# kvcache-ai/ktransformers

Hardware: NVIDIA H100
Metric: decode tok/s DeepSeek-V3 671B INT4 (Q4_K_M) MoE-block hot path; HBM GB/s vs roofline (higher is better)
Workload: dtype int8xint4/int6->int32 dp4a, fp32 scales+accumulate, bf16 in/out

## Files before the change

### include/ktb200.h

```cpp
#ifndef KTB200_H
#define KTB200_H
#include <stddef.h>
#include <stdint.h>
#ifdef __cplusplus
extern "C" {
#endif

#define KTB200_OK 0
#define KTB200_EINVAL (-1)
#define KTB200_ECUDA (-2)
#define KTB200_ESTATE (-3)
#define KTB200_ENOMEM (-4)

enum ktb200_ggml_type {
    KTB200_TYPE_F32 = 0, KTB200_TYPE_F16 = 1, KTB200_TYPE_Q8_0 = 8, KTB200_TYPE_Q2_K = 10,
    KTB200_TYPE_Q3_K = 11, KTB200_TYPE_Q4_K = 12, KTB200_TYPE_Q5_K = 13, KTB200_TYPE_Q6_K = 14,
    KTB200_TYPE_Q8_K = 15, KTB200_TYPE_IQ4_XS = 23, KTB200_TYPE_BF16 = 30,
    KTB200_TYPE_IQ2_XXS = 16, KTB200_TYPE_IQ1_S = 19,
    KTB200_TYPE_RAWINT4_G32 = 256
};

const char* ktb200_last_error(void);
const char* ktb200_version(void);
long ktb200_type_size(int ggml_type);
// ... 149 lines not shown
    void* out;
} ktb200_mla_prefill_params;
int ktb200_mla_prefill(const ktb200_mla_prefill_params* p, void* stream);
void ktb200_debug_grouped(long long* trace_dev);

int ktb200_add_rmsnorm(void* residual_dev, const void* delta_dev, const void* weight_dev, float eps, void* out_dev, int n_tokens,
                       int hidden, void* stream);
int ktb200_mla_prep(const void* q_dev, int num_heads, int qk_nope_head_dim, const void* kv_a_out_dev, const void* kv_a_norm_weight_dev,
                    float eps, const float* cos_dev, const float* sin_dev, void* kv_cache_dev, int page_size, const int* page_idx_dev,
                    const int* page_offset_dev, void* q_pe_out_dev, int n_tokens, void* stream);

int ktb200_mla_absorb_q(const void* q_dev, long q_head_stride, long q_token_stride, const void* w_uk_dev, int num_heads, int qk_nope_head_dim,
                        int kv_lora_rank, void* q_abs_out_dev, int n_tokens, void* stream);
int ktb200_mla_absorb_o(const void* attn_latent_dev, const void* w_uv_dev, int num_heads, int v_head_dim, int kv_lora_rank, void* out_dev,
                        int n_tokens, void* stream);

int ktb200_mla_kv_write(void* kv_cache, int page_size, const void* ckv, const void* k_pe, const int* page_idx,
                        const int* page_offset, int n_tokens, void* stream);

int ktb200_debug_stream_read(const void* src_dev, long bytes, int mode, int unroll, int ctas_per_sm, int chunk_bytes,
                             void* stream, float* ms_out);
void ktb200_debug_block_trace(unsigned long long* trace_dev);
long ktb200_debug_block_sync_words(ktb200_moe* moe, unsigned* host_out, long n);

#ifdef __cplusplus
}
#endif
#endif
```

### ktransformers_b200/csrc/common.cuh

```cuda
#pragma once
#include <cuda_bf16.h>
#include <cuda_fp16.h>
#include <cuda_runtime.h>
#include <stdint.h>

#include "../../include/ktb200.h"

#define QK_K 256
#define SZ_Q8_0 34
#define SZ_Q2_K 84
#define SZ_Q3_K 110
#define SZ_Q4_K 144
#define SZ_Q5_K 176
#define SZ_Q6_K 210
#define SZ_Q8_K 292
#define SZ_IQ4_XS 136
#define SZ_IQ2_XXS 66
#define SZ_IQ1_S 50
#define SZ_RAWINT4 144

namespace ktb {

void set_error(const char* fmt, ...);
void count_launch(int n = 1);
// ... 70 lines not shown
__host__ __device__ inline bool is_hidden_type(int t) {
    return t == KTB200_TYPE_F32 || t == KTB200_TYPE_F16 || t == KTB200_TYPE_BF16;
}
__host__ __device__ inline long row_bytes(long n, int t) { return n / blck_size(t) * type_size(t); }

#ifdef __CUDACC__
__device__ __forceinline__ uint4 ldg_stream16(const void* p) {
    uint4 r;
    asm volatile("ld.global.nc.L1::no_allocate.v4.u32 {%0, %1, %2, %3}, [%4];"
                 : "=r"(r.x), "=r"(r.y), "=r"(r.z), "=r"(r.w)
                 : "l"(p));
    return r;
}
__device__ __forceinline__ uint32_t ldg_stream4(const void* p) {
    uint32_t r;
    asm volatile("ld.global.nc.L1::no_allocate.u32 %0, [%1];" : "=r"(r) : "l"(p));
    return r;
}
__device__ __forceinline__ void prefetch_l2_bulk(const void* p, uint32_t bytes) {
    asm volatile("cp.async.bulk.prefetch.L2.global [%0], %1;" ::"l"(p), "r"(bytes) : "memory");
}
__device__ __forceinline__ void griddep_launch_dependents() { asm volatile("griddepcontrol.launch_dependents;" ::: "memory"); }
__device__ __forceinline__ void griddep_wait() { asm volatile("griddepcontrol.wait;" ::: "memory"); }
__device__ __forceinline__ uint16_t ldg_u16(const void* p) { return __ldg(reinterpret_cast<const unsigned short*>(p)); }
__device__ __forceinline__ uint8_t ldg_u8(const void* p) { return __ldg(reinterpret_cast<const unsigned char*>(p)); }

__device__ __forceinline__ int dp4a_s8s8(uint32_t a, uint32_t b, int c) { return __dp4a((int)a, (int)b, c); }
__device__ __forceinline__ int dp4a_u8s8(uint32_t a, uint32_t b, int c) {
    int d;
    asm("dp4a.u32.s32 %0, %1, %2, %3;" : "=r"(d) : "r"(a), "r"(b), "r"(c));
    return d;
}

__device__ __forceinline__ float warp_sum(float v) {
#pragma unroll
    for (int o = 16; o > 0; o >>= 1) v += __shfl_xor_sync(0xffffffffu, v, o);
    return v;
}

__device__ __forceinline__ float fp16_bits_to_f32(uint16_t h) { return __half2float(__ushort_as_half(h)); }

__device__ __forceinline__ uint16_t f32_to_bf16_ggml(float f) {
    uint32_t i = __float_as_uint(f);
    if ((i & 0x7fffffffu) > 0x7f800000u) return (uint16_t)((i >> 16) | 64);
    if (!(i & 0x7f800000u)) return (uint16_t)((i & 0x80000000u) >> 16);
    return (uint16_t)((i + (0x7fffu + ((i >> 16) & 1))) >> 16);
// ... 45 lines not shown
```

### ktransformers_b200/csrc/gate.cuh

```cuda
#pragma once
#include "common.cuh"

namespace ktb {

constexpr int kGateWarps = 4;
constexpr int kGateThreads = kGateWarps * 32;
constexpr int kGateTokTile = 8;

struct GateParams {
    const float* W;
    const void* x;
    int hidden_type, E, H, T, S;
    int top_k, n_group, topk_group, scoring, topk_method, norm_topk_prob;
    float routed_scaling_factor;
    const float* bias;
    float* partial;
    float* logits_out;
    int64_t* idx;
    float* w;
    const int* bsz;
    unsigned* ticket;
};

static inline int gate_splits(int E, int H, int nsms) {
// ... 6 lines not shown

__device__ __forceinline__ unsigned fkey(float f) {
    const unsigned u = __float_as_uint(f);
    return (u & 0x80000000u) ? ~u : (u | 0x80000000u);
}

constexpr int kGateEPT = 4;

__device__ __forceinline__ float fkey_inv(unsigned k) {
    return __uint_as_float((k & 0x80000000u) ? (k & 0x7fffffffu) : ~k);
}

template <int BAR>
__device__ __forceinline__ void gate_sync() {
    if (BAR == 0) __syncthreads();
    else asm volatile("bar.sync %0, %1;" ::"n"(BAR), "n"(kGateThreads) : "memory");
}
struct GateSel {
    int E, S, top_k, n_group, topk_group, scoring, topk_method, norm_topk_prob;
    float routed_scaling_factor;
    const float* bias;
    const float* partial;
};
template <int BAR>
__device__ void gate_select_token(const GateParams& pin, int t, float* sm, int64_t* idx_out, float* w_out, float* logits_out) {
    const GateSel p{pin.E, pin.S, pin.top_k, pin.n_group, pin.topk_group, pin.scoring, pin.topk_method, pin.norm_topk_prob,
                    pin.routed_scaling_factor, pin.bias, pin.partial};
    const int E = p.E, tid = threadIdx.x, lane = tid & 31, warp = tid >> 5;
    float* scores = sm;
    float* choice = sm + E;
    float* gsc = choice + E;
    unsigned* wbest = reinterpret_cast<unsigned*>(gsc + 32);
    float* red = reinterpret_cast<float*>(wbest + 2 * kGateWarps);

    float v[kGateEPT], pv[8][kGateEPT];
#pragma unroll
    for (int s = 0; s < 8; s++) {
        const float* pp = p.partial + ((long)t * p.S + s) * E;
#pragma unroll
        for (int i = 0; i < kGateEPT; i++) {
            const int e = tid + kGateThreads * i;
            pv[s][i] = (s < p.S && e < E) ? __ldcg(pp + e) : 0.f;
        }
    }
    float bv[kGateEPT];
#pragma unroll
    for (int i = 0; i < kGateEPT; i++) {
        const int e = tid + kGateThreads * i;
        bv[i] = (p.topk_method == 0 && p.bias && e < E) ? __ldg(p.bias + e) : 0.f;
    }
#pragma unroll
    for (int i = 0; i < kGateEPT; i++) {
        v[i] = 0.f;
#pragma unroll
        for (int s = 0; s < 8; s++)
            if (s < p.S) v[i] += pv[s][i];
    }
    if (logits_out) {
#pragma unroll
        for (int i = 0; i < kGateEPT; i++) {
            const int e = tid + kGateThreads * i;
            if (e < E) logits_out[(long)t * E + e] = v[i];
        }
    }
    if (p.scoring == 0) {
// ... 147 lines not shown
```

### ktransformers_b200/csrc/handles.cuh

```cuda
#pragma once
#include "common.cuh"

namespace ktb {
enum FmtId { FMT_Q4K, FMT_Q5K, FMT_Q6K8, FMT_Q6K4T, FMT_GENK, FMT_RAWINT4, FMT_NONE };
enum Q6Layout { LAYOUT_RAW = 0, LAYOUT_SOA8 = 1, LAYOUT_T4 = 2 };

static inline FmtId pick_fmt(int type, int layout) {
    if (type == KTB200_TYPE_Q4_K) return FMT_Q4K;
    if (type == KTB200_TYPE_Q5_K) return FMT_Q5K;
    if (type == KTB200_TYPE_Q6_K && layout == LAYOUT_SOA8) return FMT_Q6K8;
    if (type == KTB200_TYPE_Q6_K && layout == LAYOUT_T4) return FMT_Q6K4T;
    if (is_kquant(type) || is_iquant(type)) return FMT_GENK;
    if (is_rawint4(type)) return FMT_RAWINT4;
    return FMT_NONE;
}
}

struct ktb200_mlp {
    int H, I, gate_type, up_type, down_type, hidden_type, group_max_len, device;
    const void *gate, *up, *down;
    bool loaded, gu_soa;
    int down_layout;
    float* inter;
};

struct ktb200_moe {
    ktb200_moe_config cfg;
    int device;
    bool loaded;
    bool gu_soa;
    int down_layout;
    float* inter;
    int64_t* ids_d;
    float* w_d;
    void* in_d;
    void* out_d;
    float* blk_partial;
    unsigned* blk_sync;
    unsigned blk_flip;
    float* blk_inter;
    uint8_t* blk_stage;
    const void* pf[3];
    size_t pf_bytes[3];
};

namespace ktb {
constexpr int kBlockMaxTokens = 8;
constexpr int kBlkStatusWord = 4, kBlkReadyWord = 8;
static inline size_t blk_ready_words(const ktb200_moe_config& c) {
    const int t = c.group_max_len < kBlockMaxTokens ? c.group_max_len : kBlockMaxTokens;
    return (size_t)t * (c.routed_expert_num + 1) * (c.intermediate_size / QK_K);
}
}

struct DeviceGuard {
    int prev;
    bool ok;
    explicit DeviceGuard(int dev) : prev(0), ok(true) {
        if (cudaGetDevice(&prev) != cudaSuccess) ok = false;
        if (ok && prev != dev && cudaSetDevice(dev) != cudaSuccess) ok = false;
// ... 5 lines not shown
```

### ktransformers_b200/csrc/moe.cu

```cuda
#include <cstdio>
#include <cstdlib>
#include <cstring>
#include <new>

#define KTB_IQ_CODEBOOKS
#include "gemv_bulk.cuh"
#include "dense_bulk.cuh"
#include "rawint4.cuh"
#include "iq.cuh"
#include "handles.cuh"

namespace ktb {

__global__ void __launch_bounds__(256) repack_q6k_kernel(uint8_t* w, long n_groups, int nb) {
    extern __shared__ __align__(16) uint8_t smem[];
    const long gbytes = 8L * SZ_Q6_K * nb;
    for (long g = blockIdx.x; g < n_groups; g += gridDim.x) {
        uint8_t* base = w + g * gbytes;
        for (long i = threadIdx.x; i < gbytes / 16; i += blockDim.x)
            reinterpret_cast<uint4*>(smem)[i] = reinterpret_cast<const uint4*>(base)[i];
        __syncthreads();
        const uint16_t* src = reinterpret_cast<const uint16_t*>(smem);
        uint16_t* dst = reinterpret_cast<uint16_t*>(base);
        const long s_qh = 1024L * nb, s_sc = 1536L * nb, s_d = 1664L * nb;
// ... 551 lines not shown
        return KTB200_EINVAL;
    }
    if (!n_i4 && (!expert_type_ok(c->gate_type) || !expert_type_ok(c->up_type) || !expert_type_ok(c->down_type))) {
        set_error("MOEConfig: unsupported ggml weight type (gate %d up %d down %d)", c->gate_type, c->up_type, c->down_type);
        return KTB200_EINVAL;
    }
    if (!is_hidden_type(c->hidden_type)) { set_error("MOEConfig: hidden_type %d must be F32/F16/BF16", c->hidden_type); return KTB200_EINVAL; }
    if (c->hidden_size % QK_K || c->intermediate_size % QK_K) {
        set_error("MOEConfig: hidden_size %d and intermediate_size %d must be multiples of 256 for K-quant tensors",
                  c->hidden_size, c->intermediate_size);
        return KTB200_EINVAL;
    }
    if (!c->gate_proj || !c->up_proj || !c->down_proj) { set_error("MOEConfig: null weight pointer"); return KTB200_EINVAL; }
    DeviceGuard g(device);
    if (!g.ok) { set_error("cudaSetDevice(%d) failed", device); return KTB200_ECUDA; }
    ktb200_moe* m = new (std::nothrow) ktb200_moe();
    if (!m) return KTB200_ENOMEM;
    m->cfg = *c;
    m->device = device;
    m->loaded = false;
    m->gu_soa = false;
    m->down_layout = LAYOUT_RAW;
    m->inter = nullptr; m->ids_d = nullptr; m->w_d = nullptr; m->in_d = nullptr; m->out_d = nullptr;
    m->blk_partial = nullptr; m->blk_sync = nullptr; m->blk_flip = 0; m->blk_inter = nullptr; m->blk_stage = nullptr;
    for (int r = 0; r < 3; r++) { m->pf[r] = nullptr; m->pf_bytes[r] = 0; }
    const size_t slots = (size_t)c->group_max_len * c->routed_expert_num;
    const size_t hid = (size_t)c->group_max_len * c->hidden_size * type_size(c->hidden_type);
    cudaError_t e = cudaMalloc(&m->inter, (slots + c->group_max_len) * c->intermediate_size * sizeof(float));
    if (e == cudaSuccess) e = cudaMalloc(&m->ids_d, slots * sizeof(int64_t));
    if (e == cudaSuccess) e = cudaMalloc(&m->w_d, slots * sizeof(float));
    if (e == cudaSuccess) e = cudaMalloc(&m->in_d, hid);
    if (e == cudaSuccess) e = cudaMalloc(&m->out_d, hid);
    if (e == cudaSuccess) e = cudaMalloc(&m->blk_partial, (size_t)8 * 8 * 512 * sizeof(float));
    const size_t sync_words = kBlkReadyWord + 2 * blk_ready_words(*c);
    if (e == cudaSuccess) e = cudaMalloc(&m->blk_sync, sync_words * sizeof(unsigned));
    if (e == cudaSuccess) e = cudaMemset(m->blk_sync, 0, sync_words * sizeof(unsigned));
    if (e == cudaSuccess) e = cudaMalloc(&m->blk_inter, blk_ready_words(*c) * QK_K * sizeof(float));
    if (e == cudaSuccess) e = cudaMemset(m->blk_inter, 0xff, blk_ready_words(*c) * QK_K * sizeof(float));
    if (e == cudaSuccess) e = cudaMalloc(&m->blk_stage, blk_ready_words(*c) * (QK_K + 32 + 4));
    if (e != cudaSuccess) {
        set_error("cudaMalloc failed: %s", cudaGetErrorString(e));
        ktb200_moe_destroy(m);
        return KTB200_ENOMEM;
    }
    *out = m;
    return KTB200_OK;
}

void ktb200_moe_destroy(ktb200_moe* m) {
    if (!m) return;
    DeviceGuard g(m->device);
    cudaFree(m->inter); cudaFree(m->ids_d); cudaFree(m->w_d); cudaFree(m->in_d); cudaFree(m->out_d);
    cudaFree(m->blk_partial); cudaFree(m->blk_sync); cudaFree(m->blk_inter); cudaFree(m->blk_stage);
    delete m;
}

int ktb200_moe_load_weights(ktb200_moe* m, void* stream) {
    if (!m) { set_error("null handle"); return KTB200_EINVAL; }
    if (m->loaded) return KTB200_OK;
    DeviceGuard g(m->device);
    const ktb200_moe_config& c = m->cfg;
    cudaStream_t s = (cudaStream_t)stream;
    if (c.gate_type == KTB200_TYPE_Q6_K && c.up_type == KTB200_TYPE_Q6_K && c.intermediate_size % 8 == 0) {
        int rc = repack_q6k(const_cast<void*>(c.gate_proj), (long)c.expert_num * c.intermediate_size, c.hidden_size, m->device, s);
        if (rc) return rc;
        rc = repack_q6k(const_cast<void*>(c.up_proj), (long)c.expert_num * c.intermediate_size, c.hidden_size, m->device, s);
        if (rc) return rc;
        m->gu_soa = true;
    }
    if (c.down_type == KTB200_TYPE_Q6_K && q6k4t_eligible(c.hidden_size, c.intermediate_size, c.routed_expert_num + 1, m->device)) {
        int rc = repack_q6k4t(const_cast<void*>(c.down_proj), (long)c.expert_num * c.hidden_size, c.intermediate_size, m->device, s);
        if (rc) return rc;
        m->down_layout = LAYOUT_T4;
    } else if (c.down_type == KTB200_TYPE_Q6_K && c.hidden_size % 8 == 0) {
        int rc = repack_q6k(const_cast<void*>(c.down_proj), (long)c.expert_num * c.hidden_size, c.intermediate_size, m->device, s);
        if (rc) return rc;
// ... 330 lines not shown
```

### ktransformers_b200/csrc/moe_block.cu

```cuda
#include <cstdlib>

#include "gate.cuh"
#include "gemv_bulk.cuh"
#include "handles.cuh"

namespace ktb {

constexpr int kBlockWarps = 15;
constexpr int kBlockWarpsLo = 12;

struct BlockParams {
    GateParams g;
    const void *w_gate, *w_up, *w_down;
    const void *s_gate, *s_up, *s_down;
    int n_local, id_offset;
    int H, I, k;
    int hidden_type, use_silu;
    float* inter;
    void* out;
    unsigned* sync;
    unsigned* ready;
    unsigned* status;
    uint8_t* stage_q;
    int16_t* stage_bs;
    float* stage_d;
    int nrows_max;
    int region_a;
    int ring_bytes;
    int prime_u, prime_d;
    unsigned long long* trace;
    const uint8_t* pf[3];
    unsigned pf_bytes[3];
};

__device__ __forceinline__ unsigned ld_acquire_u32(const unsigned* p) {
    unsigned v;
    asm volatile("ld.acquire.gpu.global.u32 %0, [%1];" : "=r"(v) : "l"(p) : "memory");
    return v;
}
__device__ __forceinline__ unsigned ld_acquire_sys_u32(const unsigned* p) {
    unsigned v;
    asm volatile("ld.acquire.sys.global.u32 %0, [%1];" : "=r"(v) : "l"(p) : "memory");
    return v;
}
__device__ __forceinline__ unsigned long long ep_now() {
    unsigned long long t;
    asm volatile("mov.u64 %0, %%globaltimer;" : "=l"(t));
    return t;
}
constexpr unsigned long long kEpTimeoutNs = 4000000000ull;
template <bool SYS>
__device__ __forceinline__ void wait_ge(const unsigned* p, unsigned target, unsigned* status) {
    unsigned long long t0 = 0;
    unsigned spins = 0;
    while ((int)((SYS ? ld_acquire_sys_u32(p) : ld_acquire_u32(p)) - target) < 0) {
        if ((++spins & 1023u) == 0) {
            const unsigned long long t = ep_now();
            if (!t0) t0 = t;
            else if (t - t0 > kEpTimeoutNs) { *status = 1; break; }
        }
    }
}

__device__ __forceinline__ void grid_arrive(unsigned* counter, unsigned& gen) {
    __syncthreads();
    gen++;
    if (threadIdx.x == 0) {
        __threadfence();
        atomicAdd(counter, 1u);
    }
}
__device__ __forceinline__ void grid_wait(unsigned* counter, unsigned gen) {
    if (threadIdx.x == 0) {
// ... 55 lines not shown
    L.ring_off = ((size_t)kBlockSharedBytes + p.region_a + (size_t)p.nrows_max * ns * 4 + 15) & ~(size_t)15;
    return L;
}

__device__ __forceinline__ void blk_quantize_x(int t) {
    extern __shared__ __align__(16) uint8_t smem[];
    const BlockParams& p = reinterpret_cast<const BlockShared*>(smem)->prm;
    const BlockLay L = block_layout<8>(p, smem);
    const int lane = threadIdx.x & 31, warp = threadIdx.x >> 5, W = blockDim.x >> 5, nblk = p.H / QK_K;
    float cur[8], nxt[8];
    int b = warp;
    if (b < nblk) load_block8(p.g.x, (long)t * p.H + (long)b * QK_K + lane * 8, p.hidden_type, cur);
#pragma unroll 1
    while (b < nblk) {
        const int bn = b + W;
        if (bn < nblk) load_block8(p.g.x, (long)t * p.H + (long)bn * QK_K + lane * 8, p.hidden_type, nxt);
        warp_quantize_q8k_block(cur, lane, reinterpret_cast<uint32_t*>(L.xq + (size_t)b * kActBlkStride), L.xdx + b, nullptr, L.xbs + b * 8);
#pragma unroll
        for (int i = 0; i < 8; i++) cur[i] = nxt[i];
        b = bn;
    }
}

__device__ __forceinline__ void blk_router(int t, bool& waited) {
    extern __shared__ __align__(16) uint8_t smem[];
    const BlockParams& p = reinterpret_cast<const BlockShared*>(smem)->prm;
    const int lane = threadIdx.x & 31, warp = threadIdx.x >> 5, W = blockDim.x >> 5;
    const int E = p.g.E, S = p.g.S, n4 = p.H / 4;
    const int gw = blockIdx.x * W + warp, tw = gridDim.x * W;
    for (int u = gw; u < E * S; u += tw) {
        const int s = u / E, e = u - s * E;
        const int c0 = (int)((long)n4 * s / S), nc4 = (int)((long)n4 * (s + 1) / S) - c0;
        const float4* wrow = reinterpret_cast<const float4*>(p.g.W + (long)e * p.H) + c0;
        const long xbase = (long)t * n4 + c0;
        float acc = 0.f;
        constexpr int NQ = 10;
        for (int cb = lane; cb < nc4; cb += 32 * NQ) {
            float4 w[NQ], xv[NQ];
#pragma unroll
            for (int q = 0; q < NQ; q++) {
                const int c = cb + 32 * q;
                if (c < nc4) w[q] = __ldg(wrow + c);
            }
            if (!waited) { griddep_wait(); waited = true; }
#pragma unroll
            for (int q = 0; q < NQ; q++) {
                const int c = cb + 32 * q;
                if (c < nc4) xv[q] = load_x4(p.g.x, xbase + c, p.hidden_type);
            }
#pragma unroll
            for (int q = 0; q < NQ; q++) {
                const int c = cb + 32 * q;
                if (c < nc4) {
                    acc = fmaf(w[q].x, xv[q].x, acc);
                    acc = fmaf(w[q].y, xv[q].y, acc);
                    acc = fmaf(w[q].z, xv[q].z, acc);
                    acc = fmaf(w[q].w, xv[q].w, acc);
                }
            }
        }
        const float v = warp_sum(acc);
        if (lane == 0) p.g.partial[((long)t * S + s) * E + e] = v;
    }
    if (!waited) { griddep_wait(); waited = true; }
}

__device__ __forceinline__ void blk_select(int t) {
    extern __shared__ __align__(16) uint8_t smem[];
    BlockShared& sh = *reinterpret_cast<BlockShared*>(smem);
    const BlockParams& p = sh.prm;
    const BlockLay L = block_layout<8>(p, smem);
    const int k = p.k;
    if ((threadIdx.x >> 5) < kGateWarps) {
        gate_select_token<1>(p.g, t, L.sel, sh.ids, sh.w, blockIdx.x == 0 ? p.g.logits_out : nullptr);
    }
    __syncthreads();
    block_stamp(p, 10);
    if (threadIdx.x == 0) {
        unsigned sk = 0;
        int nv = p.s_gate ? 1 : 0;
        for (int j = 0; j < k; j++) {
            const long e = (long)sh.ids[j] - p.id_offset;
            if (e < 0 || e >= p.n_local) sk |= 1u << j; else sh.vs[nv++] = j;
        }
        sh.nv = nv;
        sh.skip = sk;
    }
    if (blockIdx.x == 0 && threadIdx.x < k) {
        p.g.idx[(long)t * k + threadIdx.x] = sh.ids[threadIdx.x];
        p.g.w[(long)t * k + threadIdx.x] = sh.w[threadIdx.x];
    }
    __syncthreads();
}

__device__ __forceinline__ void entry_slice(int I, int ie, int& r0, int& len) {
    const unsigned s = (blockIdx.x + (unsigned)ie) % gridDim.x;
    r0 = (int)((unsigned long long)I * s / gridDim.x);
    len = (int)((unsigned long long)I * (s + 1) / gridDim.x) - r0;
}

constexpr unsigned kInterEmpty = 0xffffffffu;
__device__ __forceinline__ void st_relaxed_f32(float* p, float v) {
    asm volatile("st.relaxed.gpu.global.f32 [%0], %1;" ::"l"(p), "f"(v) : "memory");
}
__device__ __forceinline__ uint4 ld_relaxed_u4(const void* p) {
    uint4 v;
    asm volatile("ld.relaxed.gpu.global.v4.u32 {%0, %1, %2, %3}, [%4];" : "=r"(v.x), "=r"(v.y), "=r"(v.z), "=r"(v.w) : "l"(p) : "memory");
    return v;
}

template <int KBS>
__device__ __forceinline__ void quantise_block(const BlockParams& p, long gb, float* src) {
    const int lane = threadIdx.x & 31;
    uint4 v0, v1;
    unsigned long long t0 = 0;
    for (unsigned spins = 1;; spins++) {
        v0 = ld_relaxed_u4(src + lane * 8);
        v1 = ld_relaxed_u4(src + lane * 8 + 4);
        const bool here = v0.x != kInterEmpty && v0.y != kInterEmpty && v0.z != kInterEmpty && v0.w != kInterEmpty &&
                          v1.x != kInterEmpty && v1.y != kInterEmpty && v1.z != kInterEmpty && v1.w != kInterEmpty;
        if (__all_sync(0xffffffffu, here)) break;
        if ((spins & 255u) == 0) {
            const unsigned long long t = ep_now();
            if (!t0) t0 = t;
            else if (t - t0 > kEpTimeoutNs) { if (lane == 0) *p.status = 1; break; }
        }
    }
// ... 98 lines not shown
    if (p.g.bsz) { griddep_wait(); waited = true; Teff = min(Teff, *p.g.bsz); }
    const int k = p.k;
    const bool has_shared = p.s_gate != nullptr;
    uint32_t bar_u32, ring_u32;
    {
        const BlockLay L = block_layout<DownFmt::kBs>(p, smem);
        const int bar_bytes = (W * SU * 8 + 15) & ~15;
        bar_u32 = (uint32_t)__cvta_generic_to_shared(smem + L.ring_off) + warp * SU * 8;
        ring_u32 = (uint32_t)__cvta_generic_to_shared(smem + L.ring_off + bar_bytes) + warp * p.ring_bytes;
    }
    if (lane == 0) {
#pragma unroll
        for (int s = 0; s < SU; s++) mbar_init(bar_u32 + 8 * s, 1);
        mbar_fence_init();
        fence_proxy_async_smem();
    }
    {
        const uint32_t* src = reinterpret_cast<const uint32_t*>(&p);
        uint32_t* dst = reinterpret_cast<uint32_t*>(&sh.prm);
        for (int i = threadIdx.x; i < (int)(sizeof(BlockParams) / 4); i += blockDim.x) dst[i] = src[i];
    }
    if (threadIdx.x == 0 && has_shared) sh.vs[0] = k;
    uint32_t phase = 0;
    unsigned gen = 0;
    block_stamp(p, 0);

  for (int t = 0; t < Teff; t++) {
    __syncthreads();
    {
        const int nblk = p.H / QK_K, row_bytes = nblk * SZ_Q4_K;
        const int ns = k + (has_shared ? 1 : 0);
        int ie = 0, ir = 0, ir0 = 0, ilen = 0, ileft = 0, isub = 0;
        int ce = 0, cr = 0, cr0 = 0, clen = 0, cleft = 0, csub = 0;
        int stride = W, iend = 1;
        int slot_i = 0, slot_u = 0;
        auto advance = [&](int& e, int& r, int& r0, int& len, int n) {
            int off = r - r0 + n;
            while (off >= len && e + 1 < iend) { off -= len; e++; entry_slice(p.I, e, r0, len); }
            r = r0 + off;
        };
        auto start_list = [&](int e0, int e1, int first, int count, int stride_) {
            iend = e1;
            ie = e0;
            entry_slice(p.I, e0, ir0, ilen);
            ir = ir0;
            advance(ie, ir, ir0, ilen, first);
            ce = ie; cr = ir; cr0 = ir0; clen = ilen;
// ... 5 lines not shown
                if (lane == 0) {
                    const int s = sh.vs[ie];
                    const bool second = isub & 1;
                    const uint8_t* src;
                    if (s == k) {
                        src = reinterpret_cast<const uint8_t*>(second ? p.s_up : p.s_gate) + (long)ir * row_bytes;
                    } else {
                        const long e = (long)sh.ids[s] - p.id_offset;
                        src = reinterpret_cast<const uint8_t*>(second ? p.w_up : p.w_gate) + (e * p.I + ir) * row_bytes;
                    }
                    const uint32_t bar = bar_u32 + 8 * slot_i;
                    mbar_expect_tx(bar, (uint32_t)row_bytes);
                    bulk_g2s(ring_u32 + slot_i * row_bytes, src, (uint32_t)row_bytes, bar);
                }
                isub++;
                if (!(isub & 1)) {
                    ileft--;
                    advance(ie, ir, ir0, ilen, stride);
                }
                slot_i = (slot_i + 1 == SU) ? 0 : slot_i + 1;
            }
        };
        if (threadIdx.x < 36) sh.ent_state[threadIdx.x] = 0;
        blk_router(t, waited);
        block_stamp(p, 2);
        grid_arrive(p.sync, gen);
        if (has_shared && warp >= kGateWarps) {
            int r0, nr;
            entry_slice(p.I, 0, r0, nr);
            const int first = warp - kGateWarps, st = W - kGateWarps;
            start_list(0, 1, first, (nr - first + st - 1) / st, st);
        }
#pragma unroll
        for (int s = 0; s < SU; s++)
            if (s < p.prime_u) issue_u();
        blk_quantize_x(t);
        block_stamp(p, 1);
        grid_wait(p.sync, gen);
        block_stamp(p, 3);
        const BlockLay L = block_layout<DownFmt::kBs>(p, smem);
        const uint8_t* ring = smem + (ring_u32 - (uint32_t)__cvta_generic_to_shared(smem));
#pragma unroll 1
        for (int list = 0; list < 2; list++) {
            if (list == 1) {
                blk_select(t);
                block_stamp(p, 4);
                const int e0 = has_shared ? 1 : 0, nv = sh.nv;
                int total = 0;
                for (int e = e0; e < nv; e++) {
                    int r0, len;
                    entry_slice(p.I, e, r0, len);
                    total += len;
                }
                start_list(e0, nv, warp, (total - warp + W - 1) / W, W);
#pragma unroll
                for (int s = 0; s < SU; s++) issue_u();
            }
            float acc_first = 0.f;
            while (cleft > 0) {
                mbar_wait(bar_u32 + 8 * slot_u, (phase >> slot_u) & 1u);
                phase ^= 1u << slot_u;
                const uint8_t* row0 = ring + slot_u * row_bytes;
                float acc = 0.f;
                if (lane < nblk)
                    acc = q4k_block_dot(row0 + lane * SZ_Q4_K, L.xq + (size_t)lane * kActBlkStride,
                                        *reinterpret_cast<const uint4*>(L.xbs + lane * 8), L.xdx[lane]);
                __syncwarp();
                slot_u = (slot_u + 1 == SU) ? 0 : slot_u + 1;
// ... 84 lines not shown
                res = warp_reduce4(acc[0], acc[1], acc[2], acc[3], lane);
            }
            __syncwarp();
            dslot_u = (dslot_u + 1 == SD) ? 0 : dslot_u + 1;
            dcons++;
            issue_d();
            if ((lane & 7) == 0) L.partial[(eq * RW + (lane >> 3)) * ns + j] = res;
            eq += Wd;
            while (eq >= nquads) { eq -= nquads; evi++; }
        }
        __syncthreads();
        block_stamp(p, 8);
        blk_combine<DownFmt::kBs>(t);
        block_stamp(p, 9);
    }
  }

    __syncthreads();
    if (threadIdx.x == 0) sh.last_cta = atomicAdd(p.sync + 1, 1u) == gridDim.x - 1;
    __syncthreads();
    if (sh.last_cta) {
        const int nready = Teff * (k + (has_shared ? 1 : 0)) * (p.I / QK_K);
        for (int i = threadIdx.x; i < nready; i += blockDim.x) p.ready[i] = 0;
        if (threadIdx.x == 0) {
            p.sync[0] = 0;
            p.sync[1] = 0;
        }
        __threadfence();
    }
}


constexpr int kEpWorldMax = 8;
constexpr int kEpPairsMax = 64;

struct EpExtra {
    int rank, world, phase_mask, pa;
    int msg_bytes;
    int inter_shared_row;
    float* shared_out;
    uint8_t* msg[kEpWorldMax];
    float* part[kEpWorldMax];
    unsigned* flags[kEpWorldMax];
    int ep_off;
};
struct EpParams { BlockParams b; EpExtra x; };

struct EpShared {
    EpExtra x;
    unsigned epoch;
// ... 424 lines not shown
        const size_t aqb = (size_t)ns * nb * (kActBlkStride + 2 * kbs + 4);
        p.region_a = (int)(((xq > aqb ? xq : aqb) + 15) & ~(size_t)15);
        size_t base = (size_t)kBlockSharedBytes + p.region_a + (size_t)p.nrows_max * ns * 4;
        base = (base + 15) & ~(size_t)15;
        static const int want_w = [] { const char* e = getenv("KTB200_BLK_WARPS"); return e ? atoi(e) : kBlockWarpsLo; }();
        const int su = want_w > kBlockWarpsLo ? 3 : 4;
        size_t ring = su * row > 2 * item ? su * row : 2 * item;
        p.ring_bytes = (int)ring;
        W = base + 64 < 232448 - 1024 ? (int)((232448 - 1024 - base - 16) / (ring + 8 * su)) : 0;
        if (W > (want_w > kBlockWarpsLo ? kBlockWarps : kBlockWarpsLo)) W = want_w > kBlockWarpsLo ? kBlockWarps : kBlockWarpsLo;
        if (want_w >= 8 && W > want_w) W = want_w;
        if (want_w > kBlockWarpsLo && W <= kBlockWarpsLo) W = 0;
        smem = base + (((size_t)W * su * 8 + 15) & ~(size_t)15) + (size_t)W * ring;
        if (W < 8 || c.hidden_size % 4 || item % 16 || c.intermediate_size < 1) fused = false;
    }
    if (!fused) {
        int rc = ktb200_moe_gate_forward(gc, qlen, input, idx, w, nullptr, bsz, stream);
        if (rc) return rc;
        return ktb200_moe_forward_shared(m, sh, qlen, k, idx, w, input, output, bsz, stream);
    }

    const int S = gate_splits(gc->n_experts, gc->hidden_size, num_sms(dev));
    p.g = GateParams{gc->weight, input, gc->hidden_type, gc->n_experts, gc->hidden_size, qlen, S, k, gc->n_group, gc->topk_group,
                     gc->scoring, gc->topk_method, gc->norm_topk_prob, gc->routed_scaling_factor, gc->bias, m->blk_partial, nullptr,
                     idx, w, bsz, nullptr};
    p.w_gate = c.gate_proj; p.w_up = c.up_proj; p.w_down = c.down_proj;
    p.s_gate = sh ? sh->gate : nullptr; p.s_up = sh ? sh->up : nullptr; p.s_down = sh ? sh->down : nullptr;
    p.n_local = c.expert_num; p.id_offset = c.expert_id_offset;
    p.H = c.hidden_size; p.I = c.intermediate_size; p.k = k; p.hidden_type = c.hidden_type; p.use_silu = c.use_silu;
    const unsigned flip = m->blk_flip++ & 1u;
    p.inter = m->blk_inter; p.out = output; p.sync = m->blk_sync + 2 * flip; p.trace = g_btrace;
    p.status = m->blk_sync + kBlkStatusWord;
    p.ready = m->blk_sync + kBlkReadyWord + flip * blk_ready_words(c);
    p.stage_q = m->blk_stage;
    p.stage_bs = reinterpret_cast<int16_t*>(m->blk_stage + blk_ready_words(c) * (size_t)QK_K);
    p.stage_d = reinterpret_cast<float*>(m->blk_stage + blk_ready_words(c) * (size_t)(QK_K + 32));
    for (int r = 0; r < 3; r++) { p.pf[r] = (const uint8_t*)m->pf[r]; p.pf_bytes[r] = (unsigned)m->pf_bytes[r]; }
    static const int prime_u = [] { const char* e = getenv("KTB200_BLK_PRIME_U"); return e ? atoi(e) : 3; }();
    p.prime_u = prime_u;

    void* args[] = {&p};
    const void* fn;
    if (W > kBlockWarpsLo) fn = fd == FMT_Q6K4T ? (const void*)moe_block_kernel<BulkQ6K4T, kBlockWarps> : (const void*)moe_block_kernel<BulkQ4K, kBlockWarps>;
    else fn = fd == FMT_Q6K4T ? (const void*)moe_block_kernel<BulkQ6K4T, kBlockWarpsLo> : (const void*)moe_block_kernel<BulkQ4K, kBlockWarpsLo>;
    static const int coop = [] { const char* e = getenv("KTB200_BLK_COOP"); return e ? atoi(e) : 1; }();
    static const int pdl = [] { const char* e = getenv("KTB200_BLK_PDL"); return e ? atoi(e) : 1; }();
    auto separate = [&]() -> int {
        int rc = ktb200_moe_gate_forward(gc, qlen, input, idx, w, nullptr, bsz, stream);
        if (rc) return rc;
        return ktb200_moe_forward_shared(m, sh, qlen, k, idx, w, input, output, bsz, stream);
    };
    {
        static size_t limit[4][64] = {};
        static int resident[4][64] = {};
        const int v = (W > kBlockWarpsLo ? 2 : 0) + (fd == FMT_Q6K4T ? 1 : 0);
        if (limit[v][dev & 63] < smem) {
            KTB_CUDA_CHECK(cudaFuncSetAttribute(fn, cudaFuncAttributeMaxDynamicSharedMemorySize, (int)smem));
            int per_sm = 0;
            KTB_CUDA_CHECK(cudaOccupancyMaxActiveBlocksPerMultiprocessor(&per_sm, fn, W * 32, smem));
            resident[v][dev & 63] = per_sm * num_sms(dev);
            limit[v][dev & 63] = smem;
        }
// ... 165 lines not shown
    if (rc) return rc;
    if (out_dev == m->out_d) KTB_CUDA_CHECK(cudaMemcpyAsync(output, m->out_d, hid, cudaMemcpyDeviceToHost, s));
    if (idx) KTB_CUDA_CHECK(cudaMemcpyAsync(idx, m->ids_d, (size_t)qlen * k * sizeof(int64_t), cudaMemcpyDeviceToHost, s));
    if (w) KTB_CUDA_CHECK(cudaMemcpyAsync(w, m->w_d, (size_t)qlen * k * sizeof(float), cudaMemcpyDeviceToHost, s));
    KTB_CUDA_CHECK(cudaStreamSynchronize(s));
    return KTB200_OK;
}

extern "C" void ktb200_debug_block_trace(unsigned long long* trace_dev) { g_btrace = trace_dev; }

extern "C" long ktb200_debug_block_sync_words(ktb200_moe* m, unsigned* host_out, long n) {
    if (!m) { set_error("null handle"); return -1; }
    const long total = (long)(kBlkReadyWord + 2 * blk_ready_words(m->cfg));
    DeviceGuard guard(m->device);
    if (host_out && n > 0) {
        if (cudaDeviceSynchronize() != cudaSuccess ||
            cudaMemcpy(host_out, m->blk_sync, (size_t)(n < total ? n : total) * sizeof(unsigned), cudaMemcpyDeviceToHost) != cudaSuccess) {
            set_error("debug_block_sync_words: %s", cudaGetErrorString(cudaGetLastError()));
            return -1;
        }
    }
    return total;
}
```

### ktransformers_b200/native.py

```python
from __future__ import annotations

import ctypes as C
import os
import subprocess
import threading

_HERE = os.path.dirname(os.path.abspath(__file__))
LIB_PATH = os.path.join(_HERE, "libktb200.so")
CSRC = os.path.join(_HERE, "csrc")

OK, EINVAL, ECUDA, ESTATE, ENOMEM = 0, -1, -2, -3, -4

GGML_F32, GGML_F16, GGML_Q8_0, GGML_Q2_K, GGML_Q3_K, GGML_Q4_K, GGML_Q5_K, GGML_Q6_K, GGML_Q8_K = 0, 1, 8, 10, 11, 12, 13, 14, 15
GGML_IQ4_XS, GGML_BF16 = 23, 30
GGML_IQ2_XXS, GGML_IQ1_S = 16, 19
RAWINT4_G32 = 256


class MoeConfig(C.Structure):
    _fields_ = [("expert_num", C.c_int), ("routed_expert_num", C.c_int), ("hidden_size", C.c_int),
                ("intermediate_size", C.c_int), ("stride", C.c_int), ("group_min_len", C.c_int),
                ("group_max_len", C.c_int), ("use_silu", C.c_int), ("gate_proj", C.c_void_p), ("up_proj", C.c_void_p),
                ("down_proj", C.c_void_p), ("gate_type", C.c_int), ("up_type", C.c_int), ("down_type", C.c_int),
                ("hidden_type", C.c_int), ("expert_id_offset", C.c_int)]
# ... 50 lines not shown
    "ktb200_linear_load_weights": (_I, [_VP, _VP]),
    "ktb200_linear_forward": (_I, [_VP, _I, _VP, _VP, _VP, _VP, _VP]),
    "ktb200_mlp_create": (_I, [_I, _I, _VP, _VP, _VP, _I, _I, _I, _I, _I, _I, C.POINTER(_VP)]),
    "ktb200_mlp_destroy": (None, [_VP]),
    "ktb200_mlp_load_weights": (_I, [_VP, _VP]),
    "ktb200_mlp_forward": (_I, [_VP, _I, _VP, _VP, _I, _VP, _VP]),
    "ktb200_moe_forward_shared": (_I, [_VP, _VP, _I, _I, _VP, _VP, _VP, _VP, _VP, _VP]),
    "ktb200_quantize_activations": (_I, [_VP, _I, _L, _L, _I, _VP, _VP]),
    "ktb200_dequantize": (_I, [_VP, _I, _L, _VP, _I, _VP]),
    "ktb200_rawint4_pack": (_I, [_VP, _VP, _L, _L, _VP, _VP]),
    "ktb200_moe_gate_forward": (_I, [C.POINTER(GateConfig), _I, _VP, _VP, _VP, _VP, _VP, _VP]),
    "ktb200_moe_block_forward": (_I, [C.POINTER(GateConfig), _VP, _VP, _I, _VP, _VP, _VP, _VP, _VP, _VP]),
    "ktb200_moe_block_forward_host": (_I, [C.POINTER(GateConfig), _VP, _VP, _I, _VP, _VP, _VP, _VP, _VP]),
    "ktb200_moe_forward_ep": (_I, [_VP, _VP, _I, _I, _VP, _VP, _VP, _VP, _I, _VP, _VP, _VP]),
    "ktb200_ep_all_gather_tokens": (_I, [_VP, _VP, _VP, _VP]),
    "ktb200_ep_reduce_own_token": (_I, [_VP, _VP, _VP, _VP]),
    "ktb200_moe_block_prefetch_hint": (_I, [_VP, _VP, _VP, _I]),
    "ktb200_ep_msg_bytes": (_L, [_I, _I]),
    "ktb200_moe_ep_block_forward": (_I, [_VP, _VP, _VP, _VP, _VP, _VP, _VP, _VP, _I, _VP]),
    "ktb200_ep_tokens_layout": (_L, [_I, _I, _I, _I, _I, _VP]),
    "ktb200_moe_ep_forward_tokens": (_I, [_VP, _VP, _VP, _VP, _VP, _VP, _VP, _VP, _VP, _I, _VP]),
    "ktb200_debug_block_trace": (None, [_VP]),
    "ktb200_debug_block_sync_words": (_L, [_VP, _VP, _L]),
    "ktb200_debug_stream_read": (_I, [_VP, _L, _I, _I, _I, _I, _VP, C.POINTER(C.c_float)]),
    "ktb200_mla_workspace_bytes": (C.c_size_t, [_I, _I, _I]),
    "ktb200_mla_decode": (_I, [C.POINTER(MlaParams), _VP]),
    "ktb200_debug_mla": (None, [_VP]),
    "ktb200_mla_prefill": (_I, [C.POINTER(MlaPrefillParams), _VP]),
    "ktb200_debug_grouped": (None, [_VP]),
    "ktb200_mla_absorb_q": (_I, [_VP, _L, _L, _VP, _I, _I, _I, _VP, _I, _VP]),
    "ktb200_mla_absorb_o": (_I, [_VP, _VP, _I, _I, _I, _VP, _I, _VP]),
    "ktb200_add_rmsnorm": (_I, [_VP, _VP, _VP, C.c_float, _VP, _I, _I, _VP]),
    "ktb200_mla_prep": (_I, [_VP, _I, _I, _VP, _VP, C.c_float, _VP, _VP, _VP, _I, _VP, _VP, _VP, _I, _VP]),
    "ktb200_mla_kv_write": (_I, [_VP, _I, _VP, _VP, _VP, _VP, _I, _VP]),
}


class EpComm(C.Structure):
    _fields_ = [("rank", C.c_int), ("world", C.c_int), ("hidden_size", C.c_int), ("hidden_type", C.c_int),
                ("token_bufs", C.POINTER(C.c_void_p)), ("partial_bufs", C.POINTER(C.c_void_p)), ("flag_bufs", C.POINTER(C.c_void_p))]

    @classmethod
    def make(cls, rank, world, hidden_size, hidden_type, tok_ptrs, part_ptrs, flag_ptrs):
        arr = lambda ps: (C.c_void_p * world)(*[int(x) for x in ps])
        c = cls(rank, world, hidden_size, hidden_type)
        c._keep = (arr(tok_ptrs), arr(part_ptrs), arr(flag_ptrs))
# ... 73 lines not shown
```

### profiles/block_trace.py

```python
#!/usr/bin/env python
import ctypes as C
import os
import sys

sys.path.insert(0, os.path.dirname(os.path.dirname(os.path.abspath(__file__))))
import numpy as np
import torch

from ktransformers_b200 import native
from ktransformers_b200.util.synth import synth_blocks

lib = native.lib()
E, K, H, I = 256, 8, 7168, 2048
Q4_K, Q6_K, BF16 = 12, 14, 30
S = lambda: torch.cuda.current_stream().cuda_stream
layers = []
for l in range(3):
    g, u, d = synth_blocks(Q4_K, E * I * H, device="cuda", seed=3 * l), synth_blocks(Q4_K, E * I * H, device="cuda", seed=3 * l + 1), synth_blocks(Q6_K, E * H * I, device="cuda", seed=3 * l + 2)
    sg, su, sd = synth_blocks(Q4_K, I * H, device="cuda", seed=100 + l), synth_blocks(Q4_K, I * H, device="cuda", seed=200 + l), synth_blocks(Q6_K, H * I, device="cuda", seed=300 + l)
    cfg = native.MoeConfig(E, K, H, I, 64, 10, 8, 1, g.data_ptr(), u.data_ptr(), d.data_ptr(), Q4_K, Q4_K, Q6_K, BF16, 0)
    moe = C.c_void_p(); native.check(lib.ktb200_moe_create(C.byref(cfg), 0, C.byref(moe))); native.check(lib.ktb200_moe_load_weights(moe, S()))
    mlp = C.c_void_p(); native.check(lib.ktb200_mlp_create(H, I, sg.data_ptr(), su.data_ptr(), sd.data_ptr(), Q4_K, Q4_K, Q6_K, BF16, 8, 0, C.byref(mlp)))
    native.check(lib.ktb200_mlp_load_weights(mlp, S()))
    W = torch.randn(E, H, device="cuda"); b = torch.randn(E, device="cuda")
    gc = native.GateConfig(E, H, K, 8, 4, 0, 0, 1, 2.5, W.data_ptr(), b.data_ptr(), BF16)
    layers.append((gc, moe, mlp, (g, u, d, sg, su, sd, W, b)))
x = (torch.randn(1, H, device="cuda") / 100).to(torch.bfloat16)
y = torch.zeros(1, H, dtype=torch.bfloat16, device="cuda")
ids = torch.zeros(1, K, dtype=torch.int64, device="cuda"); wts = torch.zeros(1, K, device="cuda")
n_sm = torch.cuda.get_device_properties(torch.cuda.current_device()).multi_processor_count
trace = torch.zeros(n_sm * 16, dtype=torch.int64, device="cuda")
names = ["start", "x quantised (under barrier 1)", "router partials written", "grid barrier 1 passed", "top-k selected",
         "gate/up done (CTA)", "entry 0 ready (its a in smem)", "last entry ready (its a in smem)", "down tiles done (CTA)", "combined + stored",
         "  (top-k done, before the work-list build)"]
acc = []
for rep in range(12):
    gc, moe, mlp, _ = layers[rep % 3]
    lib.ktb200_debug_block_trace(trace.data_ptr())
    native.check(lib.ktb200_moe_block_forward(C.byref(gc), moe, mlp, 1, x.data_ptr(), y.data_ptr(), ids.data_ptr(), wts.data_ptr(), None, S()))
    torch.cuda.synchronize()
    t = trace.cpu().numpy().reshape(n_sm, 16)[:, :11].astype(np.float64)
    t -= t[:, 0].min()
    if rep >= 3:
        acc.append(t)
lib.ktb200_debug_block_trace(None)
t = np.mean(acc, axis=0) / 1e3
print(f"{'boundary':42s} {'first':>8s} {'median':>8s} {'last':>8s}   (us after the first CTA started; mean of {len(acc)} launches)")
for i in sorted(range(len(names)), key=lambda i: np.median(t[:, i])):
    print(f"{names[i]:42s} {t[:, i].min():8.2f} {np.median(t[:, i]):8.2f} {t[:, i].max():8.2f}")
```

Measured before the change: 160.2.

## Replace router grid barrier with per-element sentinel polling on router partials

Removes the grid-wide barrier between router partial computation and top-k selection. Each CTA now polls the partial logits in a dedicated buffer until no entry holds the 0xffffffff sentinel. The last CTA resets the buffer to the sentinel after use, and partials are written with relaxed stores. All shared-expert up-prefetch issues now go out before the router work, replacing the env-tunable prime count. This trades a global barrier for redundant polling loads and adds a cleanup pass, plus a timeout path for safety.

```diff
diff --git a/include/ktb200.h b/include/ktb200.h
--- a/include/ktb200.h
+++ b/include/ktb200.h
@@ -195,6 +195,7 @@
                              void* stream, float* ms_out);
 void ktb200_debug_block_trace(unsigned long long* trace_dev);
 long ktb200_debug_block_sync_words(ktb200_moe* moe, unsigned* host_out, long n);
+long ktb200_debug_block_partial_words(ktb200_moe* moe, unsigned* host_out, long n);
 
 #ifdef __cplusplus
 }
diff --git a/ktransformers_b200/csrc/common.cuh b/ktransformers_b200/csrc/common.cuh
--- a/ktransformers_b200/csrc/common.cuh
+++ b/ktransformers_b200/csrc/common.cuh
@@ -116,6 +116,12 @@
 }
 __device__ __forceinline__ void griddep_launch_dependents() { asm volatile("griddepcontrol.launch_dependents;" ::: "memory"); }
 __device__ __forceinline__ void griddep_wait() { asm volatile("griddepcontrol.wait;" ::: "memory"); }
+__device__ __forceinline__ unsigned long long ep_now() {
+    unsigned long long t;
+    asm volatile("mov.u64 %0, %%globaltimer;" : "=l"(t));
+    return t;
+}
+constexpr unsigned long long kEpTimeoutNs = 4000000000ull;
 __device__ __forceinline__ uint16_t ldg_u16(const void* p) { return __ldg(reinterpret_cast<const unsigned short*>(p)); }
 __device__ __forceinline__ uint8_t ldg_u8(const void* p) { return __ldg(reinterpret_cast<const unsigned char*>(p)); }
 
diff --git a/ktransformers_b200/csrc/gate.cuh b/ktransformers_b200/csrc/gate.cuh
--- a/ktransformers_b200/csrc/gate.cuh
+++ b/ktransformers_b200/csrc/gate.cuh
@@ -52,8 +52,16 @@
     const float* bias;
     const float* partial;
 };
-template <int BAR>
-__device__ void gate_select_token(const GateParams& pin, int t, float* sm, int64_t* idx_out, float* w_out, float* logits_out) {
+constexpr unsigned kInterEmpty = 0xffffffffu;
+__device__ __forceinline__ float ld_relaxed_f32(const float* p) {
+    float v;
+    asm volatile("ld.relaxed.gpu.global.f32 %0, [%1];" : "=f"(v) : "l"(p) : "memory");
+    return v;
+}
+
+template <int BAR, bool POLL = false>
+__device__ void gate_select_token(const GateParams& pin, int t, float* sm, int64_t* idx_out, float* w_out, float* logits_out,
+                                  unsigned* status = nullptr, unsigned long long* seen = nullptr) {
     const GateSel p{pin.E, pin.S, pin.top_k, pin.n_group, pin.topk_group, pin.scoring, pin.topk_method, pin.norm_topk_prob,
                     pin.routed_scaling_factor, pin.bias, pin.partial};
     const int E = p.E, tid = threadIdx.x, lane = tid & 31, warp = tid >> 5;
@@ -64,13 +72,45 @@
     float* red = reinterpret_cast<float*>(wbest + 2 * kGateWarps);
 
     float v[kGateEPT], pv[8][kGateEPT];
-#pragma unroll
-    for (int s = 0; s < 8; s++) {
-        const float* pp = p.partial + ((long)t * p.S + s) * E;
-#pragma unroll
-        for (int i = 0; i < kGateEPT; i++) {
-            const int e = tid + kGateThreads * i;
-            pv[s][i] = (s < p.S && e < E) ? __ldcg(pp + e) : 0.f;
+    if (POLL) {
+        const float* base = p.partial + (long)t * p.S * E + tid;
+        unsigned long long t0 = 0;
+        for (unsigned spins = 1;; spins++) {
+            int Er = E;
+            asm volatile("" : "+r"(Er));
+            bool here = true;
+#pragma unroll
+            for (int s = 0; s < 8; s++) {
+#pragma unroll
+                for (int i = 0; i < kGateEPT; i++) {
+                    const int e = tid + kGateThreads * i;
+                    pv[s][i] = (s < p.S && e < E) ? ld_relaxed_f32(base + s * Er + kGateThreads * i) : 0.f;
+                }
+            }
+#pragma unroll
+            for (int s = 0; s < 8; s++)
+#pragma unroll
+                for (int i = 0; i < kGateEPT; i++) here = here && __float_as_uint(pv[s][i]) != kInterEmpty;
+            if (here) break;
+            if ((spins & 1023u) == 0) {
+                const unsigned long long now = ep_now();
+                if (!t0) t0 = now;
+                else if (now - t0 > kEpTimeoutNs) { *status = 1; break; }
+            }
+        }
+        if (seen) {
+            gate_sync<BAR>();
+            if (tid == 0) *seen = ep_now();
+        }
+    } else {
+#pragma unroll
+        for (int s = 0; s < 8; s++) {
+            const float* pp = p.partial + ((long)t * p.S + s) * E;
+#pragma unroll
+            for (int i = 0; i < kGateEPT; i++) {
+                const int e = tid + kGateThreads * i;
+                pv[s][i] = (s < p.S && e < E) ? __ldcg(pp + e) : 0.f;
+            }
         }
     }
     float bv[kGateEPT];
diff --git a/ktransformers_b200/csrc/handles.cuh b/ktransformers_b200/csrc/handles.cuh
--- a/ktransformers_b200/csrc/handles.cuh
+++ b/ktransformers_b200/csrc/handles.cuh
@@ -36,6 +36,7 @@
     void* in_d;
     void* out_d;
     float* blk_partial;
+    float* blk_rpart;
     unsigned* blk_sync;
     unsigned blk_flip;
     float* blk_inter;
diff --git a/ktransformers_b200/csrc/moe.cu b/ktransformers_b200/csrc/moe.cu
--- a/ktransformers_b200/csrc/moe.cu
+++ b/ktransformers_b200/csrc/moe.cu
@@ -597,7 +597,7 @@
     m->gu_soa = false;
     m->down_layout = LAYOUT_RAW;
     m->inter = nullptr; m->ids_d = nullptr; m->w_d = nullptr; m->in_d = nullptr; m->out_d = nullptr;
-    m->blk_partial = nullptr; m->blk_sync = nullptr; m->blk_flip = 0; m->blk_inter = nullptr; m->blk_stage = nullptr;
+    m->blk_partial = nullptr; m->blk_rpart = nullptr; m->blk_sync = nullptr; m->blk_flip = 0; m->blk_inter = nullptr; m->blk_stage = nullptr;
     for (int r = 0; r < 3; r++) { m->pf[r] = nullptr; m->pf_bytes[r] = 0; }
     const size_t slots = (size_t)c->group_max_len * c->routed_expert_num;
     const size_t hid = (size_t)c->group_max_len * c->hidden_size * type_size(c->hidden_type);
@@ -607,6 +607,8 @@
     if (e == cudaSuccess) e = cudaMalloc(&m->in_d, hid);
     if (e == cudaSuccess) e = cudaMalloc(&m->out_d, hid);
     if (e == cudaSuccess) e = cudaMalloc(&m->blk_partial, (size_t)8 * 8 * 512 * sizeof(float));
+    if (e == cudaSuccess) e = cudaMalloc(&m->blk_rpart, (size_t)kBlockMaxTokens * 8 * 512 * sizeof(float));
+    if (e == cudaSuccess) e = cudaMemset(m->blk_rpart, 0xff, (size_t)kBlockMaxTokens * 8 * 512 * sizeof(float));
     const size_t sync_words = kBlkReadyWord + 2 * blk_ready_words(*c);
     if (e == cudaSuccess) e = cudaMalloc(&m->blk_sync, sync_words * sizeof(unsigned));
     if (e == cudaSuccess) e = cudaMemset(m->blk_sync, 0, sync_words * sizeof(unsigned));
@@ -626,7 +628,7 @@
     if (!m) return;
     DeviceGuard g(m->device);
     cudaFree(m->inter); cudaFree(m->ids_d); cudaFree(m->w_d); cudaFree(m->in_d); cudaFree(m->out_d);
-    cudaFree(m->blk_partial); cudaFree(m->blk_sync); cudaFree(m->blk_inter); cudaFree(m->blk_stage);
+    cudaFree(m->blk_partial); cudaFree(m->blk_rpart); cudaFree(m->blk_sync); cudaFree(m->blk_inter); cudaFree(m->blk_stage);
     delete m;
 }
 
diff --git a/ktransformers_b200/csrc/moe_block.cu b/ktransformers_b200/csrc/moe_block.cu
--- a/ktransformers_b200/csrc/moe_block.cu
+++ b/ktransformers_b200/csrc/moe_block.cu
@@ -43,12 +43,6 @@
     asm volatile("ld.acquire.sys.global.u32 %0, [%1];" : "=r"(v) : "l"(p) : "memory");
     return v;
 }
-__device__ __forceinline__ unsigned long long ep_now() {
-    unsigned long long t;
-    asm volatile("mov.u64 %0, %%globaltimer;" : "=l"(t));
-    return t;
-}
-constexpr unsigned long long kEpTimeoutNs = 4000000000ull;
 template <bool SYS>
 __device__ __forceinline__ void wait_ge(const unsigned* p, unsigned target, unsigned* status) {
     unsigned long long t0 = 0;
@@ -150,6 +144,11 @@
     }
 }
 
+__device__ __forceinline__ void st_relaxed_f32(float* p, float v) {
+    asm volatile("st.relaxed.gpu.global.f32 [%0], %1;" ::"l"(p), "f"(v) : "memory");
+}
+
+template <bool RELAXED = false>
 __device__ __forceinline__ void blk_router(int t, bool& waited) {
     extern __shared__ __align__(16) uint8_t smem[];
     const BlockParams& p = reinterpret_cast<const BlockShared*>(smem)->prm;
@@ -188,11 +187,15 @@
             }
         }
         const float v = warp_sum(acc);
-        if (lane == 0) p.g.partial[((long)t * S + s) * E + e] = v;
+        if (lane == 0) {
+            if (RELAXED) st_relaxed_f32(p.g.partial + ((long)t * S + s) * E + e, v);
+            else p.g.partial[((long)t * S + s) * E + e] = v;
+        }
     }
     if (!waited) { griddep_wait(); waited = true; }
 }
 
+template <bool POLL = false>
 __device__ __forceinline__ void blk_select(int t) {
     extern __shared__ __align__(16) uint8_t smem[];
     BlockShared& sh = *reinterpret_cast<BlockShared*>(smem);
@@ -200,7 +203,8 @@
     const BlockLay L = block_layout<8>(p, smem);
     const int k = p.k;
     if ((threadIdx.x >> 5) < kGateWarps) {
-        gate_select_token<1>(p.g, t, L.sel, sh.ids, sh.w, blockIdx.x == 0 ? p.g.logits_out : nullptr);
+        gate_select_token<1, POLL>(p.g, t, L.sel, sh.ids, sh.w, blockIdx.x == 0 ? p.g.logits_out : nullptr, p.status,
+                                   POLL && p.trace ? p.trace + blockIdx.x * 16 + 3 : nullptr);
     }
     __syncthreads();
     block_stamp(p, 10);
@@ -227,10 +231,6 @@
     len = (int)((unsigned long long)I * (s + 1) / gridDim.x) - r0;
 }
 
-constexpr unsigned kInterEmpty = 0xffffffffu;
-__device__ __forceinline__ void st_relaxed_f32(float* p, float v) {
-    asm volatile("st.relaxed.gpu.global.f32 [%0], %1;" ::"l"(p), "f"(v) : "memory");
-}
 __device__ __forceinline__ uint4 ld_relaxed_u4(const void* p) {
     uint4 v;
     asm volatile("ld.relaxed.gpu.global.v4.u32 {%0, %1, %2, %3}, [%4];" : "=r"(v.x), "=r"(v.y), "=r"(v.z), "=r"(v.w) : "l"(p) : "memory");
@@ -375,7 +375,6 @@
     }
     if (threadIdx.x == 0 && has_shared) sh.vs[0] = k;
     uint32_t phase = 0;
-    unsigned gen = 0;
     block_stamp(p, 0);
 
   for (int t = 0; t < Teff; t++) {
@@ -427,9 +426,6 @@
             }
         };
         if (threadIdx.x < 36) sh.ent_state[threadIdx.x] = 0;
-        blk_router(t, waited);
-        block_stamp(p, 2);
-        grid_arrive(p.sync, gen);
         if (has_shared && warp >= kGateWarps) {
             int r0, nr;
             entry_slice(p.I, 0, r0, nr);
@@ -437,18 +433,18 @@
             start_list(0, 1, first, (nr - first + st - 1) / st, st);
         }
 #pragma unroll
-        for (int s = 0; s < SU; s++)
-            if (s < p.prime_u) issue_u();
+        for (int s = 0; s < SU; s++) issue_u();
+        blk_router<true>(t, waited);
+        block_stamp(p, 2);
         blk_quantize_x(t);
         block_stamp(p, 1);
-        grid_wait(p.sync, gen);
-        block_stamp(p, 3);
+        __syncthreads();
         const BlockLay L = block_layout<DownFmt::kBs>(p, smem);
         const uint8_t* ring = smem + (ring_u32 - (uint32_t)__cvta_generic_to_shared(smem));
 #pragma unroll 1
         for (int list = 0; list < 2; list++) {
             if (list == 1) {
-                blk_select(t);
+                blk_select<true>(t);
                 block_stamp(p, 4);
                 const int e0 = has_shared ? 1 : 0, nv = sh.nv;
                 int total = 0;
@@ -579,10 +575,9 @@
     if (sh.last_cta) {
         const int nready = Teff * (k + (has_shared ? 1 : 0)) * (p.I / QK_K);
         for (int i = threadIdx.x; i < nready; i += blockDim.x) p.ready[i] = 0;
-        if (threadIdx.x == 0) {
-            p.sync[0] = 0;
-            p.sync[1] = 0;
-        }
+        const int npart = Teff * p.g.S * p.g.E;
+        for (int i = threadIdx.x; i < npart; i += blockDim.x) reinterpret_cast<unsigned*>(p.g.partial)[i] = kInterEmpty;
+        if (threadIdx.x == 0) p.sync[1] = 0;
         __threadfence();
     }
 }
@@ -1053,7 +1048,7 @@
 
     const int S = gate_splits(gc->n_experts, gc->hidden_size, num_sms(dev));
     p.g = GateParams{gc->weight, input, gc->hidden_type, gc->n_experts, gc->hidden_size, qlen, S, k, gc->n_group, gc->topk_group,
-                     gc->scoring, gc->topk_method, gc->norm_topk_prob, gc->routed_scaling_factor, gc->bias, m->blk_partial, nullptr,
+                     gc->scoring, gc->topk_method, gc->norm_topk_prob, gc->routed_scaling_factor, gc->bias, m->blk_rpart, nullptr,
                      idx, w, bsz, nullptr};
     p.w_gate = c.gate_proj; p.w_up = c.up_proj; p.w_down = c.down_proj;
     p.s_gate = sh ? sh->gate : nullptr; p.s_up = sh ? sh->up : nullptr; p.s_down = sh ? sh->down : nullptr;
@@ -1067,8 +1062,6 @@
     p.stage_bs = reinterpret_cast<int16_t*>(m->blk_stage + blk_ready_words(c) * (size_t)QK_K);
     p.stage_d = reinterpret_cast<float*>(m->blk_stage + blk_ready_words(c) * (size_t)(QK_K + 32));
     for (int r = 0; r < 3; r++) { p.pf[r] = (const uint8_t*)m->pf[r]; p.pf_bytes[r] = (unsigned)m->pf_bytes[r]; }
-    static const int prime_u = [] { const char* e = getenv("KTB200_BLK_PRIME_U"); return e ? atoi(e) : 3; }();
-    p.prime_u = prime_u;
 
     void* args[] = {&p};
     const void* fn;
@@ -1280,3 +1273,17 @@
     }
     return total;
 }
+
+extern "C" long ktb200_debug_block_partial_words(ktb200_moe* m, unsigned* host_out, long n) {
+    if (!m) { set_error("null handle"); return -1; }
+    const long total = (long)kBlockMaxTokens * 8 * 512;
+    DeviceGuard guard(m->device);
+    if (host_out && n > 0) {
+        if (cudaDeviceSynchronize() != cudaSuccess ||
+            cudaMemcpy(host_out, m->blk_rpart, (size_t)(n < total ? n : total) * sizeof(unsigned), cudaMemcpyDeviceToHost) != cudaSuccess) {
+            set_error("debug_block_partial_words: %s", cudaGetErrorString(cudaGetLastError()));
+            return -1;
+        }
+    }
+    return total;
+}
diff --git a/ktransformers_b200/native.py b/ktransformers_b200/native.py
--- a/ktransformers_b200/native.py
+++ b/ktransformers_b200/native.py
@@ -96,6 +96,7 @@
     "ktb200_moe_ep_forward_tokens": (_I, [_VP, _VP, _VP, _VP, _VP, _VP, _VP, _VP, _VP, _I, _VP]),
     "ktb200_debug_block_trace": (None, [_VP]),
     "ktb200_debug_block_sync_words": (_L, [_VP, _VP, _L]),
+    "ktb200_debug_block_partial_words": (_L, [_VP, _VP, _L]),
     "ktb200_debug_stream_read": (_I, [_VP, _L, _I, _I, _I, _I, _VP, C.POINTER(C.c_float)]),
     "ktb200_mla_workspace_bytes": (C.c_size_t, [_I, _I, _I]),
     "ktb200_mla_decode": (_I, [C.POINTER(MlaParams), _VP]),
diff --git a/profiles/block_trace.py b/profiles/block_trace.py
--- a/profiles/block_trace.py
+++ b/profiles/block_trace.py
@@ -30,7 +30,7 @@
 ids = torch.zeros(1, K, dtype=torch.int64, device="cuda"); wts = torch.zeros(1, K, device="cuda")
 n_sm = torch.cuda.get_device_properties(torch.cuda.current_device()).multi_processor_count
 trace = torch.zeros(n_sm * 16, dtype=torch.int64, device="cuda")
-names = ["start", "x quantised (under barrier 1)", "router partials written", "grid barrier 1 passed", "top-k selected",
+names = ["start", "x quantised", "router partials written", "all router partials seen", "top-k selected",
          "gate/up done (CTA)", "entry 0 ready (its a in smem)", "last entry ready (its a in smem)", "down tiles done (CTA)", "combined + stored",
          "  (top-k done, before the work-list build)"]
 acc = []
```

Result: no change. 160.2 (median of 6 runs) (-0.0%).
